# shiinamiyuki/akari_render

Hardware: AMD Instinct MI355X
Metric: Msamples/s (whole node), 1080p path tracer, C2 (higher is better)
Workload: dtype f32

## Files before the change

akari_render_amd/build.py:

```python
from __future__ import annotations

import os
import subprocess
import sys

HERE = os.path.dirname(os.path.abspath(__file__))
CSRC = os.path.join(HERE, "csrc")
LIB = os.path.join(HERE, "libakari_hip.so")

PT_KINDS = ["plain", "inst", "feat", "punct", "punct_tree"]
PT_UNITS = {"pt_unit_" + kind + ("_env" if env else "") + ("_lens" if lens else ""): 4 * k + 2 * env + lens
            for k, kind in enumerate(PT_KINDS) for env in (0, 1) for lens in (0, 1)}

SOURCES = [
    "pt_kernels.hip", "pt_kernels_relaxed.hip", *PT_UNITS, "probe_kernels.hip",
    "wf_env_kernels.hip",
    "wf_lens_kernels.hip", "aov_lens_kernels.hip",
    "wf_kernels.hip", "wf_sort.hip",
    "aov_kernels.hip", "gpt_kernels.hip", "mcmc_kernels.hip", "denoise_kernels.hip", "adapt_kernels.hip", "display_kernels.hip",
    "host/options.cpp", "host/api_common.cpp", "host/api_scene.cpp", "host/api_pt.cpp", "host/wf_schedule.cpp", "host/api_aux.cpp", "host/api_task.cpp", "host/api_probe.cpp", "host/api_denoise.cpp", "host/api_adapt.cpp", "host/api_display.cpp",
    "host/scene_build.cpp", "host/scene_inst.cpp", "host/scene_env.cpp", "host/scene_punct.cpp",
    "host/scene_json.cpp",
    "host/bvh.cpp",
    "host/image_io.cpp",
    "host/image_formats.cpp",
    "host/pmj_tables.cpp",
    "host/comm.cpp",
    "host/specialise.cpp",
]
TEST_HOOKS = os.environ.get("AKR_SHIP", "0") != "1"


def _headers():
# ... 186 lines not shown
```

akari_render_amd/capi.py:

```python
from __future__ import annotations

import ctypes as C
import os
from typing import Optional

import numpy as np

from . import abi
from .build import LIB, build

AKR_OK = 0
FILM_PLANE_RGB, FILM_PLANE_SPLAT, FILM_PLANE_WEIGHT, FILM_PLANES_PT, FILM_PLANES_ALL = 1, 2, 4, 5, 7
ERR_INVALID_ARGUMENT, ERR_HIP, ERR_NO_DEVICE, ERR_IO, ERR_PARSE, ERR_UNSUPPORTED, ERR_OOM, ERR_RENDER = -1, -2, -3, -4, -5, -6, -7, -8

(ARRAY_WOOP, ARRAY_TRI_GID, ARRAY_SHADE, ARRAY_INSTANCES, ARRAY_MATERIALS, ARRAY_BVH_NODES, ARRAY_LIGHT_ENTRIES,
 ARRAY_LIGHT_PDF, ARRAY_AREA_ENTRIES, ARRAY_AREA_PDF, ARRAY_INST_TRI_OFFSET, ARRAY_R2C, ARRAY_C2W,
 ARRAY_TEX_NODES, ARRAY_TEX_IMAGES, ARRAY_TEX_TEXELS, ARRAY_MAT_INPUTS,
 ARRAY_INST_LEAVES, ARRAY_MESH_TRIS, ARRAY_MESH_POS, ARRAY_MESH_META, ARRAY_MESH_NORMALS,
 ARRAY_ENV_MARGINAL_ENTRIES, ARRAY_ENV_MARGINAL_PDF, ARRAY_ENV_CONDITIONAL_ENTRIES, ARRAY_ENV_CONDITIONAL_PDF, ARRAY_ENV_TEXELS,
 ARRAY_PUNCTUAL_LIGHTS, ARRAY_LIGHT_TREE) = range(29)
ENV_LIGHT_INSTANCE = 0xFFFFFFFF
PUNCTUAL_LIGHT_INSTANCE = 0xFFFFFFFE
LIGHT_TREE_INSTANCE = 0xFFFFFFFD

# ... 22 lines not shown
]
TEST_EXPORTS = [
    "akr_probe_material_inputs_host", "akr_host_stdrng_u64", "akr_host_chacha_block", "akr_host_pcg32_states",
    "akr_host_pcg_start", "akr_host_alias_table", "akr_probe_math", "akr_probe_bsdf", "akr_probe_intersect",
    "akr_probe_surface_interaction", "akr_probe_material_inputs", "akr_host_decode_png", "akr_host_decode_jpeg",
    "akr_host_decode_exr", "akr_host_decode_tiff", "akr_host_decode_dds", "akr_host_pmj02bn_tables",
    "akr_probe_material_folded_host", "akr_host_sobol_dim1", "akr_host_fastmod", "akr_host_tri_pretest",
    "akr_probe_env_sample", "akr_probe_env_pdf", "akr_host_lens_ray", "akr_probe_camera_rays",
    "akr_probe_div", "akr_probe_intersect_pair", "akr_probe_math2", "akr_host_denoise", "akr_probe_denoise_times",
    "akr_host_pt_launch_plan", "akr_host_denoise_variance", "akr_probe_denoise_variance_times",
    "akr_host_tile_error", "akr_host_half_bracket", "akr_probe_adapt_times",
    "akr_host_display_transform", "akr_host_luminance_histogram", "akr_probe_display_times",
    "akr_host_pt_features_plan", "akr_host_pcg_end_pass", "akr_probe_pcg_end_pass",
    "akr_host_light_sample", "akr_probe_light_sample", "akr_host_light_sample_soft", "akr_probe_light_sample_soft",
    "akr_host_light_tree_sample", "akr_probe_light_tree_sample", "akr_host_option_info",
]


class OptionInfo(C.Structure):
    _fields_ = [("name", C.c_char_p), ("env", C.c_char_p), ("default_value", C.c_int32), ("ranged", C.c_int32), ("lo", C.c_int32), ("hi", C.c_int32)]


class RenderSession(C.Structure):

    _fields_ = [("save_intermediate", C.c_int32), ("save_stats", C.c_int32), ("name", C.c_char_p),
                ("override_sampler_independent", C.c_int32), ("verbose", C.c_int32)]


class AkariError(RuntimeError):
    def __init__(self, code: int, msg: str):
# ... 84 lines not shown
    proto("akr_film_resolve", vp, fp)
    proto("akr_film_device_ptr", vp, vpp, u64p)
    proto("akr_pt_kernel_info", vp, C.POINTER(abi.KernelInfo))
    proto("akr_scene_spec_source", vp, C.c_char_p, u64, u64p)
    proto("akr_host_spec_compile", vp, u32, u32, C.c_char_p, u64p, C.c_char_p, u32)
    proto("akr_probe_material_folded_host", vp, u32, u32, fp, up, fp, fp)
    proto("akr_host_sobol_dim1", u32, up, up, up)
    proto("akr_host_fastmod", u32, up, up, up)
    proto("akr_host_tri_pretest", u32, fp, fp, f32, up, up, fp)
    proto("akr_host_spec_compile_text", C.c_char_p, u32, u32, C.c_char_p, C.c_char_p)
    proto("akr_context_device_ordinal", vp, C.POINTER(C.c_int32))
    proto("akr_device_count", C.POINTER(C.c_int32))
    proto("akr_option_set", C.c_char_p, i32)
    proto("akr_option_get", C.c_char_p, C.POINTER(C.c_int32))
    proto("akr_host_option_info", u32, C.POINTER(OptionInfo))
    proto("akr_comm_unique_id", C.POINTER(C.c_uint8))
    proto("akr_comm_create", vp, C.POINTER(C.c_uint8), i32, i32, vpp)
    proto("akr_comm_wrap", vp, vp, i32, i32, vpp)
    proto("akr_comm_destroy", vp)
    proto("akr_film_reduce", vp, vp, i32, i32)
    proto("akr_film_reduce_planes", vp, vp, i32, i32, u32)
    proto("akr_mcmc_render_shard", vp, vp, C.POINTER(abi.McmcConfig), u32, u32, vp, C.POINTER(abi.McmcPartial), up, C.POINTER(abi.PtStats))
    proto("akr_mcmc_combine_host", vp, C.POINTER(abi.McmcPartial), u32, C.POINTER(abi.McmcResult))
    proto("akr_mcmc_combine", vp, vp, i32, C.POINTER(abi.McmcPartial), C.POINTER(abi.McmcResult))
    proto("akr_pt_config_default", C.POINTER(abi.PtConfig))
    proto("akr_aov_config_default", C.POINTER(abi.AovConfig))
    proto("akr_aov_render", vp, vp, C.POINTER(abi.AovConfig), vp, C.POINTER(abi.PtStats))
    proto("akr_gpt_config_default", C.POINTER(abi.GptConfig))
    proto("akr_gpt_render", vp, vp, C.POINTER(abi.GptConfig), vp, fp, C.POINTER(abi.PtStats))
    proto("akr_gpt_begin", vp, vp, C.POINTER(abi.GptConfig), vp, vp, vpp)
# ... 393 lines not shown


def get_option(name: str) -> int:
    v = C.c_int32()
    check(lib().akr_option_get(name.encode(), C.byref(v)))
    return v.value


def option_table() -> list:
    rows, o = [], OptionInfo()
    while lib().akr_host_option_info(len(rows), C.byref(o)) == 0:
        rows.append({"name": o.name.decode(), "env": o.env.decode(), "default": o.default_value, "range": (o.lo, o.hi) if o.ranged else None})
    return rows


class options:

    def __init__(self, **kw):
        self.kw, self.old = kw, {}

    def __enter__(self):
        for k, v in self.kw.items():
            self.old[k] = get_option(k)
            set_option(k, v)
        return self

    def __exit__(self, *exc):
        for k, v in self.old.items():
            set_option(k, v)
        return False
# ... 111 lines not shown
            self._guides = (albedo, normal)
            check(lib().akr_pt_begin_features(ctx.h if ctx is not None else None, scene.h, C.byref(self._cfg), film.h if film is not None else None,
                                              albedo.h if albedo is not None else None, normal.h if normal is not None else None, C.byref(self.h)))

    def passes(self, n: int = 1, blocking: bool = False) -> int:
        done = C.c_uint32()
        check(lib().akr_pt_passes(self.h, n, 1 if blocking else 0, C.byref(done)))
        return done.value

    def set_active_tiles(self, tiles) -> None:
        if tiles is None:
            check(lib().akr_pt_set_active_tiles(self.h, None, 0))
            return
        t = np.ascontiguousarray(tiles, dtype=np.uint32).reshape(-1)
        check(lib().akr_pt_set_active_tiles(self.h, _up(t) if t.size else C.cast(C.pointer(C.c_uint32(0)), C.POINTER(C.c_uint32)), t.size))

    def sampler_states(self, n_pixels: int) -> np.ndarray:
        st = np.zeros(2 * n_pixels, dtype=np.uint64)
        check(lib().akr_pt_read_sampler_states(self.h, st.ctypes.data_as(C.POINTER(C.c_uint64))))
        return st

    def stats(self) -> dict:
        st = abi.PtStats()
        check(lib().akr_pt_get_stats(self.h, C.byref(st)))
        return st.as_dict()

    def kernel_info(self) -> dict:
        ki = abi.KernelInfo()
        ki.struct_size = C.sizeof(abi.KernelInfo)
        check(lib().akr_pt_kernel_info(self.h, C.byref(ki)))
# ... 466 lines not shown
```

akari_render_amd/csrc/device/pt_pass.h:

```cpp
#pragma once
#include "dpath.h"

namespace akr {

#ifndef AKR_PT_MIN_WAVES
#define AKR_PT_MIN_WAVES 4
#endif
#ifndef AKR_PT_MIN_WAVES_BVH
#define AKR_PT_MIN_WAVES_BVH 4
#endif
#ifndef AKR_PT_MIN_WAVES_FD
#define AKR_PT_MIN_WAVES_FD 4
#endif
#ifndef AKR_PT_MIN_WAVES_TEX
#define AKR_PT_MIN_WAVES_TEX 3
#endif
#ifndef AKR_PT_MIN_WAVES_BVH_TEX
#define AKR_PT_MIN_WAVES_BVH_TEX 3
#endif
template <bool TEX>
using PairWalkOpt = WalkOpt<!TEX>;
template <bool BVH, bool FD, bool TEX, bool PMJ, bool STAGE, bool DEFER, uint32_t ABSENT = 0, bool INST = false, bool ENV = false, bool LENS = false, bool FEAT = false, bool PUNCT = false, bool LTREE = false>
AKR_D void pt_pass_body(const PtParams& p) {
    extern __shared__ __attribute__((aligned(16))) uint32_t lds_stack[];
// ... 11 lines not shown
        uint32_t* l = lds_stack + p.tile_offset;
        const uint32_t* g = (const uint32_t*)p.sc.bvh_nodes;
        for (uint32_t i = threadIdx.x; i < p.sc.bvh_tile_nodes * kBvhNodeWords; i += 256u) l[i] = g[i];
        __syncthreads();
    }
    const float4* lds_recs = nullptr;
    if (!BVH) {
        uint32_t* l = lds_stack + (p.stage_total >> 2);
        const uint32_t* g = (const uint32_t*)p.sc.woop;
        for (uint32_t i = threadIdx.x; i < (p.sc.n_tris + 2u) * 12u; i += 256u) l[i] = g[i];
        __syncthreads();
        lds_recs = (const float4*)l;
    }
    const uint32_t item = blockIdx.x * 256u + threadIdx.x;
    uint32_t px = 0, py = 0;
    const bool in_frame = item < p.n_items && item_to_pixel(p, item, px, py);
    const uint32_t pix = px + py * p.width;
    uint32_t sx, sy;
    shifted_pixel(p, px, py, sx, sy);
    if (PMJ && p.bn_offset != 0) pmj_bluenoise_stage(p, px, py);
    PathRegs r;
    path_regs_init<PMJ, LENS, FEAT>(r, q, in_frame, pix, sx, sy);
    constexpr bool PARK = !FD && TEX;
    uint32_t* park = lds_stack + p.park_offset + threadIdx.x;
    if (PARK) {
        park_put(park, PK_PIX, pix);
        park_put(park, PK_SX, sx);
        park_put(park, PK_SY, sy);
        if (FEAT) {
            park_put(park, PK_FEAT_A + 0, f2u(r.feat_a.x)); park_put(park, PK_FEAT_A + 1, f2u(r.feat_a.y)); park_put(park, PK_FEAT_A + 2, f2u(r.feat_a.z));
            park_put(park, PK_FEAT_N + 0, f2u(r.feat_n.x)); park_put(park, PK_FEAT_N + 1, f2u(r.feat_n.y)); park_put(park, PK_FEAT_N + 2, f2u(r.feat_n.z));
// ... 93 lines not shown
                    r.deferred = false;
                } else if (r.has_ray && found && (iteration & q.defer_metal)) {
                    const uint32_t mat = f2u(sc.shade[(size_t)hit.gid * SHADE_ROWS + 6].y);
                    if (sc.materials[mat].flags & q.defer_flags) {
                        r.d_gid = hit.gid; r.d_u = hit.u; r.d_v = hit.v;
                        r.deferred = true;
                        r.has_ray = false;
                    }
                }
            }
            if (STRAG > 0 && r.carry) {
            } else if (PARK) path_step<FD ? 1 : 0, TEX, PMJ, DEFER ? 1 : 2, ABSENT, INST, ENV, LENS, FEAT, PUNCT, LTREE>(q, r, hit, found, occluded, 0, 0, 0, park);
            else path_step<FD ? 1 : 0, TEX, PMJ, 0, ABSENT, INST, ENV, LENS, FEAT, PUNCT, LTREE>(q, r, hit, found, occluded, pix, sx, sy);
        }
    }
    flush_counters(p, r, tc.cnt, BVH);
}

constexpr int pt_pass_min_waves(bool bvh, bool fd, bool tex) {
    return bvh ? (tex ? AKR_PT_MIN_WAVES_BVH_TEX : AKR_PT_MIN_WAVES_BVH) : (fd ? AKR_PT_MIN_WAVES_FD : (tex ? AKR_PT_MIN_WAVES_TEX : AKR_PT_MIN_WAVES));
}

}
```

akari_render_amd/csrc/host/api_internal.h:

```cpp
#pragma once
#include <atomic>
#include <mutex>
#include <hip/hip_runtime.h>

#include <algorithm>
#include <array>
#include <cstdlib>
#include <cstdio>
#include <chrono>
#include <cstring>
#include <functional>
#include <map>
#include <memory>
#include <new>
#include <stdexcept>
#include <string>
#include <vector>

#include "scene_build.h"
#include "specialise.h"
#include "stdrng.h"


namespace akr_api {
// ... 164 lines not shown
struct RenderBase {
    akr_context* ctx = nullptr;
    akr_scene* scene = nullptr;
    akr_film* film = nullptr;
    akr_pt_config cfg;
    DevBuf states, counters;
    TileGrid grid;
    DevBuf owned_tiles;
    uint32_t spp_done = 0, n_launches = 0;
    uint32_t pmj_spp = 1;
    const akr_scene::ColorSet* color_set = nullptr;
    TuningOptions opt;
    std::vector<std::pair<hipEvent_t, hipEvent_t>> pending;
    double kernel_ms = 0.0;
    PtVariant variant{};
    PtParams params;
    bool holds_scene = false;
    akr_film *feat_albedo = nullptr, *feat_normal = nullptr;
    void fold_events(bool all) {
        size_t keep = 0;
        for (size_t i = 0; i < pending.size(); i++) {
            auto& ev = pending[i];
            if (all || hipEventQuery(ev.second) == hipSuccess) {
                float t = 0.0f;
                if (hipEventElapsedTime(&t, ev.first, ev.second) == hipSuccess) kernel_ms += t;
                (void)hipEventDestroy(ev.first);
                (void)hipEventDestroy(ev.second);
            } else {
                pending[keep++] = ev;
            }
// ... 27 lines not shown
    }
};

struct akr_pt_session : RenderBase {
    std::unique_ptr<WavefrontState> wf;
    int sched_trial = 0;
    uint64_t passes_launched = 0;
    bool spec_active = false;
    bool wf_sort = false;
    bool arith_relaxed = false;
    int spec_waves = 3;
    std::shared_ptr<SpecKernel> spec;
    std::string spec_status = "not requested";
    DevBuf active_tiles;
    bool active_set = false;
};

namespace akr_api {
bool choose_wavefront(const akr_pt_session* se);
std::unique_ptr<WavefrontState> wf_allocate(const akr_pt_session* se, bool sort);
void wf_set_range(WavefrontState& ws, uint32_t n_active);
void wf_run(akr_pt_session* se);
bool schedule_trial_eligible(const akr_pt_session* se);
struct LaunchTimer {
    RenderBase* se;
    hipEvent_t e0 = nullptr, e1 = nullptr;
    explicit LaunchTimer(RenderBase* s) : se(s) {
        HIP_CHECK(hipEventCreate(&e0));
        HIP_CHECK(hipEventCreate(&e1));
        HIP_CHECK(hipEventRecord(e0, se->ctx->stream));
// ... 12 lines not shown
    }
};

void base_begin(RenderBase* se, akr_context* ctx, akr_scene* scene, const akr_pt_config* cfg, akr_film* film, const TuningOptions* opt = nullptr);
int32_t render_begin(akr_context* ctx, akr_scene* scene, const akr_pt_config* cfg, akr_film* film, RenderBase** out);
int32_t base_end(RenderBase* se, akr_pt_stats* stats);
void session_params(RenderBase* se, bool spec_active = false, int spec_waves = 3);
inline void set_launch_passes(RenderBase* se, uint32_t n_passes, uint32_t last_pass_spp) {
    se->params.n_passes = n_passes;
    se->params.last_pass_spp = last_pass_spp;
}
struct PtPlan {
    PtVariant v;
    uint32_t simple_scene, defer_metal, defer_flags;
    uint32_t stage_bytes[13], stage_total, tex_slots;
};
PtPlan pt_plan(const akr_scene* s, const akr_pt_config& c, const TuningOptions& opt, bool spec_active, int spec_waves, bool feat = false);
std::string pt_features_refusal(const akr_scene* s, const TuningOptions& t);
PtVariant pt_scene_facts(const akr_scene* s, const akr_pt_config& c);
std::string pt_punctual_refusal(const akr_scene* s, const TuningOptions& t);
inline uint32_t scene_stack_depth(const CompiledScene& cs) {
    return cs.instanced.on ? cs.bvh_depth : std::max(1u, std::min(cs.bvh_depth, kBvhStackDepth));
}
inline uint32_t scene_n_nodes(const CompiledScene& cs) { return (uint32_t)((cs.instanced.on ? cs.instanced.nodes.size() : cs.bvh_nodes.size()) / kBvhNodeWords); }
void camera_params(PtParams& p, const akr_scene* s, uint32_t filter_type, float filter_radius);
template <typename End>
int32_t end_keeping_first_error(int32_t rc, End&& end) {
    const std::string err = g_last_error;
    const int32_t rc2 = end();
    if (rc == AKR_OK) return rc2;
    g_last_error = err;
    return rc;
// ... 11 lines not shown
```

akari_render_amd/csrc/host/api_probe.cpp:

```cpp
#if defined(AKR_TEST_HOOKS) && AKR_TEST_HOOKS
#include "api_internal.h"
#include "../../../include/akari_hip_test.h"
#include "../device/dinst.h"
#include "../device/disect.h"
#include "../device/dpath.h"

extern "C" {

AKR_TEST_API int32_t akr_host_stdrng_u64(uint64_t seed, uint32_t n, uint64_t* out) {
    if (!out) return fail(AKR_ERR_INVALID_ARGUMENT, "out is NULL");
    StdRng rng(seed);
    for (uint32_t i = 0; i < n; i++) out[i] = rng.next_u64();
    return AKR_OK;
}
AKR_TEST_API int32_t akr_host_chacha_block(const uint32_t* key8, uint64_t counter, uint64_t stream, int32_t rounds, uint32_t* out16) {
    if (!key8 || !out16) return fail(AKR_ERR_INVALID_ARGUMENT, "NULL argument");
    StdRng::chacha_block(key8, counter, stream, rounds, out16);
    return AKR_OK;
}
AKR_TEST_API int32_t akr_host_pcg32_states(uint64_t seed, uint64_t n, uint64_t* out2n) {
    if (!out2n) return fail(AKR_ERR_INVALID_ARGUMENT, "out is NULL");
    StdRng rng(seed);
    for (uint64_t i = 0; i < n; i++) {
        Pcg32 p = pcg_new_seq_offset(i, rng.next_u64());
// ... 345 lines not shown
        const auto vl = fill_launch_plan(scene, cfg, t, spec_waves, feat != 0, &out->plan);
        out->feat = vl.first.feat ? 1u : 0u;
        out->kernel_compiled = pt_variant_compiled(vl.first) ? 1u : 0u;
        out->park_slots = (vl.second.carry_offset - vl.second.park_offset) / 256u;
        out->required_bytes = (uint32_t)vl.second.required_bytes;
        out->lds_budget = (uint32_t)pt_lds_budget(vl.first.tex);
        out->park_slots_feat = kParkSlotsFeat;
    });
}
AKR_TEST_API int32_t akr_host_option_info(uint32_t index, akr_option_info* out) {
    OptionInfo o;
    if (!out || !tuning_info(index, &o)) return fail(AKR_ERR_INVALID_ARGUMENT, "akr_host_option_info: out is NULL or index is past the table's last row");
    *out = {o.name, o.env, o.def, o.ranged, o.lo, o.hi};
    return AKR_OK;
}
AKR_TEST_API int32_t akr_probe_camera_rays(akr_context* ctx, akr_scene* scene, uint32_t filter_type, float filter_radius, uint32_t n, const uint32_t* pixels2,
                                      const float* u4, float* out6) {
    if (!ctx || !scene || !pixels2 || !u4 || !out6) return fail(AKR_ERR_INVALID_ARGUMENT, "akr_probe_camera_rays: NULL argument");
    if (filter_type > AKR_FILTER_GAUSSIAN) return fail(AKR_ERR_INVALID_ARGUMENT, "akr_probe_camera_rays: unknown filter_type");
    return guarded([&] {
        ctx->bind();
        DevBuf dpx, du, dout;
        dpx.upload(std::vector<uint32_t>(pixels2, pixels2 + 2ull * n));
        du.upload(std::vector<float>(u4, u4 + 4ull * n));
        dout.alloc(6ull * n * 4);
        if (n) HIP_CHECK(launch_probe_camera_rays(probe_camera_params(scene, filter_type, filter_radius), n, dpx.as<uint32_t>(), du.as<float>(), dout.as<float>(), ctx->stream));
        HIP_CHECK(hipStreamSynchronize(ctx->stream));
        if (n) HIP_CHECK(hipMemcpy(out6, dout.p, 6ull * n * 4, hipMemcpyDeviceToHost));
    });
}
// ... 169 lines not shown
```

akari_render_amd/csrc/host/api_pt.cpp:

```cpp
#include "api_internal.h"

void akr_api::camera_params(PtParams& p, const akr_scene* s, uint32_t filter_type, float filter_radius) {
    std::memcpy(p.r2c, s->r2c, 64);
    std::memcpy(p.c2w, s->c2w, 64);
    p.c2w_identity = s->c2w_identity;
    p.width = s->flat.camera.width;
    p.height = s->flat.camera.height;
    p.filter_type = filter_type;
    p.filter_radius = filter_radius;
    p.lens_radius = s->flat.lens.radius;
    p.lens_focal = s->flat.lens.focal_distance;
}
PtVariant akr_api::pt_scene_facts(const akr_scene* s, const akr_pt_config& c) {
    const CompiledScene& cs = s->cs;
    PtVariant v;
    v.bvh = cs.has_tree();
    v.fd = c.force_diffuse != 0;
    v.tex = cs.has_textures;
    v.pmj = c.sampler_type != AKR_SAMPLER_INDEPENDENT;
    v.inst = cs.instanced.on;
    v.env = cs.env.on;
    v.lens = s->flat.lens.radius > 0.0f;
    v.punct = !cs.punct.empty();
    v.ltree = !cs.punct_tree.empty();
// ... 3 lines not shown
    if (s->cs.punct.empty()) return "";
    const std::string who = "a " + punctual_light_name(s->cs);
    if (t.wavefront == 1) return "unsupported: the scene has " + who + " and the wavefront schedule is forced (option wavefront = 1); only the megakernel samples punctual lights";
    if (t.arith == 1) return "unsupported: the scene has " + who + "; the relaxed arithmetic tier (option arith = 1) has no kernels that sample punctual lights";
    return "";
}
std::string akr_api::pt_features_refusal(const akr_scene* s, const TuningOptions& t) {
    if (s->cs.instanced.on)
        return "unsupported: akr_pt_begin_features: the scene is kept as meshes + instances (option instancing); its kernels collect no guides -- render them with akr_aov_render";
    if (t.wavefront == 1) return "unsupported: akr_pt_begin_features: the wavefront schedule is forced (option wavefront = 1); only the megakernel collects guides";
    if (t.arith == 1) return "unsupported: akr_pt_begin_features: the relaxed arithmetic tier (option arith = 1) has no kernels that collect guides";
    if (!s->cs.punct.empty())
        return "unsupported: akr_pt_begin_features: the scene has a " + punctual_light_name(s->cs) + "; the kernels that sample punctual lights collect no guides -- render them with akr_aov_render";
    return "";
}
PtPlan akr_api::pt_plan(const akr_scene* s, const akr_pt_config& c, const TuningOptions& opt, bool spec_active, int spec_waves, bool feat) {
    const CompiledScene& cs = s->cs;
    PtPlan pl{};
    PtVariant& v = pl.v = pt_scene_facts(s, c);
    v.feat = feat;
    const bool plain = !v.env && !v.lens && !v.feat && !v.punct;
    {
        bool simple = !cs.has_textures;
        for (const DMaterial& m : cs.materials) {
            if (m.kind == MAT_GLASS) simple = false;
            if (m.kind == MAT_PRINCIPLED && ((m.flags & (MF_COAT | MF_EVAL_DIEL | MF_NORMAL_MAP)) != 0 || m.transmission != 0.0f || m.coat_weight != 0.0f)) simple = false;
        }
        pl.simple_scene = (simple && opt.simple_kernels && plain) ? 1u : 0u;
        v.simple = pl.simple_scene != 0 && !v.fd && !v.tex && !v.inst;
    }
    {
// ... 32 lines not shown
        };
        const bool may = !v.inst && total <= (bvh ? kStageMaxBytesBvh : kStageMaxBytes);
        const size_t ggx_bytes = 4096 * sizeof(float);
        if (may && !bvh && v.tex && !v.fd && fits(total + ggx_bytes)) {
            bytes[12] = ggx_bytes;
            total += ggx_bytes;
            v.stage = true;
        } else {
            v.stage = may && (!bvh || fits(total));
        }
        if (v.stage) {
            for (int i = 0; i < 13; i++) pl.stage_bytes[i] = (uint32_t)bytes[i];
            pl.stage_total = (uint32_t)std::max<size_t>(total, 16);
        }
    }
    if (!pt_variant_compiled(v)) throw RenderError("pt_plan: no kernel for the variant decided");
    return pl;
}
void akr_api::session_params(RenderBase* se, bool spec_active, int spec_waves) {
    PtParams& p = se->params;
    const akr_scene* s = se->scene;
    const akr_pt_config& c = se->cfg;
    std::memset(&p, 0, sizeof p);
    p.sc = s->dscene;
    camera_params(p, s, c.filter_type, c.filter_radius);
    p.max_depth = c.max_depth;
    p.rr_depth = c.rr_depth;
    p.use_nee = c.use_nee;
    p.indirect_only = c.indirect_only;
    p.force_diffuse = c.force_diffuse;
// ... 19 lines not shown
    }
    p.sampler = c.sampler_type;
    if (c.sampler_type == AKR_SAMPLER_PMJ02BN || c.sampler_type == AKR_SAMPLER_SOBOL) {
        p.smp_seed = (uint32_t)c.sampler_seed;
        p.smp_spp = se->pmj_spp;
        uint32_t w = se->pmj_spp - 1;
        w |= w >> 1; w |= w >> 2; w |= w >> 4; w |= w >> 8; w |= w >> 16;
        p.smp_w = w;
        p.smp_mod_magic = fastmod_magic(se->pmj_spp);
        if (c.sampler_type == AKR_SAMPLER_PMJ02BN) {
            p.pmj_sets = se->ctx->pmj_sets.as<uint32_t>();
            p.bluenoise = se->ctx->bluenoise.as<uint16_t>();
        }
    }
    {
        const PtPlan plan = pt_plan(s, c, se->opt, spec_active, spec_waves, se->feat_albedo != nullptr);
        se->variant = plan.v;
        std::memcpy(p.stage_bytes, plan.stage_bytes, sizeof p.stage_bytes);
        p.stage_total = plan.stage_total;
        p.tex_slots = plan.tex_slots;
        p.simple_scene = plan.simple_scene;
        p.defer_metal = plan.defer_metal;
        p.defer_flags = plan.defer_flags;
    }
    for (int a = 0; a < 3; a++) {
        const float lo = s->cs.scene_lo[a], ext = s->cs.scene_hi[a] - s->cs.scene_lo[a];
        p.sort_lo[a] = lo;
        p.sort_scale[a] = ext > 0.0f ? 128.0f / ext : 0.0f;
    }
    p.shard_rank = c.shard_count > 1 ? c.shard_rank : 0;
    p.shard_count = c.shard_count > 1 ? c.shard_count : 1;
    p.tile_w = se->grid.tile_w;
// ... 6 lines not shown
    p.feat_normal = se->feat_normal ? se->feat_normal->data : nullptr;
}
std::vector<uint32_t> akr_api::owned_tiles(uint32_t tiles_x, uint32_t tiles_y, uint32_t rank, uint32_t count) {
    std::vector<std::pair<uint32_t, uint32_t>> mine;
    for (uint32_t ty = 0; ty < tiles_y; ty++)
        for (uint32_t tx = 0; tx < tiles_x; tx++)
            if (tile_owner(tx, ty, count) == rank) mine.emplace_back(tile_morton(tx, ty), ty * tiles_x + tx);
    std::sort(mine.begin(), mine.end());
    std::vector<uint32_t> out;
    out.reserve(mine.size());
    for (const auto& m : mine) out.push_back(m.second);
    return out;
}

static void read_stats(RenderBase* se, akr_pt_stats* stats);

static void validate_config(const akr_pt_config& c, const TileGrid& grid) {
    if (c.spp_per_pass == 0) throw std::invalid_argument("akr_pt_config: spp_per_pass must be > 0");
    if (c.filter_type > AKR_FILTER_GAUSSIAN) throw std::invalid_argument("akr_pt_config: unknown filter_type");
    if (c.sampler_type > AKR_SAMPLER_SOBOL) throw std::invalid_argument("akr_pt_config: unknown sampler_type");
    if (c.color > (AKR_COLOR_REPR_ACESCG | AKR_COLOR_RGB_ACESCG)) throw std::invalid_argument("akr_pt_config: unknown colour pipeline bits");
    if (c.sampler_type == AKR_SAMPLER_PMJ02BN && c.spp > 65536u)
        throw std::invalid_argument("Pmj02BnSampler supports up to 65536 spp (sampler/mod.rs:381-387)");
    if ((grid.tile_w % 8) || (grid.tile_h % 8)) throw std::invalid_argument("akr_pt_config: tile_w and tile_h must be multiples of 8");
    if (c.shard_count > 1 && c.shard_rank >= c.shard_count) throw std::invalid_argument("akr_pt_config: shard_rank >= shard_count");
    if (c.sample_begin != 0 || c.sample_count != 0) {
        if (c.sampler_type != AKR_SAMPLER_PMJ02BN && c.sampler_type != AKR_SAMPLER_SOBOL)
            throw Unsupported("akr_pt_config: a sample range needs an index-based sampler (pmj02bn, sobol): the independent sampler's start() advances the pixel's "
                              "PCG stream from wherever the previous sample stopped (sampler/mod.rs:115-131,192-203), sample s cannot be drawn without samples 0 .. s-1");
        if (c.sample_count == 0) throw std::invalid_argument("akr_pt_config: sample_begin without sample_count");
// ... 68 lines not shown
        se->states.upload(init);
    } else {
        std::vector<uint64_t> seeds(n);
        StdRng rng(cfg->sampler_seed);
        for (auto& v : seeds) v = rng.next_u64();
        DevBuf dseeds;
        dseeds.upload(seeds);
        se->states.alloc(n * sizeof(Pcg32));
        HIP_CHECK(launch_init_pcg32(dseeds.as<uint64_t>(), se->states.p, n, ctx->stream));
        HIP_CHECK(hipStreamSynchronize(ctx->stream));
    }
    se->counters.alloc(8 * kStatStripes * sizeof(uint64_t));
    HIP_CHECK(hipMemsetAsync(se->counters.p, 0, se->counters.bytes, ctx->stream));
    if (cfg->shard_count > 1) se->owned_tiles.upload(owned_tiles(se->grid.tiles_x, se->grid.tiles_y, cfg->shard_rank, cfg->shard_count));
    se->opt = opt ? *opt : tuning();
    scene->sessions++;
    se->holds_scene = true;
}
int32_t akr_api::render_begin(akr_context* ctx, akr_scene* scene, const akr_pt_config* cfg, akr_film* film, RenderBase** out) {
    *out = nullptr;
    return guarded([&] {
        auto se = std::make_unique<RenderBase>();
        base_begin(se.get(), ctx, scene, cfg, film);
        session_params(se.get());
        HIP_CHECK(hipStreamSynchronize(ctx->stream));
        *out = se.release();
    });
}
static int32_t pt_begin(akr_context* ctx, akr_scene* scene, const akr_pt_config* cfg, akr_film* film, akr_film* albedo, akr_film* normal, const TuningOptions& t, akr_pt_session** out) {
    *out = nullptr;
// ... 37 lines not shown
                se->spec_waves = t.specialise_waves ? t.specialise_waves : 3;
                se->spec_active = true;
            }
            session_params(se.get(), se->spec_active, se->spec_waves);
            if (se->spec_active) {
                se->spec = ctx->spec_cache.get(scene->spec_header, se->variant, se->spec_waves, ctx->props.gcnArchName, may_compile);
                se->spec_status = se->spec->status;
                if (!se->spec->fn) {
                    se->spec_active = false;
                    session_params(se.get(), false, se->spec_waves);
                }
            }
            se->params.wf_sort = se->wf_sort ? 1u : 0u;
        }
        if (wavefront) se->wf = wf_allocate(se.get(), se->wf_sort);
        se->sched_trial = schedule_trial_eligible(se.get()) ? 1 : 0;
        HIP_CHECK(hipStreamSynchronize(ctx->stream));
        *out = se.release();
    });
}
extern "C" {
AKR_API int32_t akr_pt_begin(akr_context* ctx, akr_scene* scene, const akr_pt_config* cfg, akr_film* film, akr_pt_session** out) {
    if (!out) return fail(AKR_ERR_INVALID_ARGUMENT, "akr_pt_begin: NULL argument");
    return pt_begin(ctx, scene, cfg, film, nullptr, nullptr, tuning(), out);
}
AKR_API int32_t akr_pt_begin_features(akr_context* ctx, akr_scene* scene, const akr_pt_config* cfg, akr_film* film, akr_film* albedo, akr_film* normal, akr_pt_session** out) {
    if (!out) return fail(AKR_ERR_INVALID_ARGUMENT, "akr_pt_begin_features: NULL argument");
    *out = nullptr;
    if (!ctx || (scene && !scene->ctx))
        return fail(AKR_ERR_UNSUPPORTED, "unsupported: akr_pt_begin_features: guides are collected by GPU kernels; a host-only scene (no device context) cannot render them");
// ... 4 lines not shown
        if (g->ctx != ctx) return fail(AKR_ERR_INVALID_ARGUMENT, "akr_pt_begin_features: a guide film belongs to another context");
        if (g->width != scene->flat.camera.width || g->height != scene->flat.camera.height)
            return fail(AKR_ERR_INVALID_ARGUMENT, "akr_pt_begin_features: a guide film's resolution does not match the scene camera");
    }
    const TuningOptions t = tuning();
    const std::string why = pt_features_refusal(scene, t);
    if (!why.empty()) return fail(AKR_ERR_UNSUPPORTED, why);
    return pt_begin(ctx, scene, cfg, film, albedo, normal, t, out);
}
AKR_API int32_t akr_pt_passes(akr_pt_session* se, uint32_t n_passes, int32_t blocking, uint32_t* spp_done) {
    if (!se) return fail(AKR_ERR_INVALID_ARGUMENT, "session is NULL");
    return guarded([&] {
        se->ctx->bind();
        uint32_t kMaxFusedPasses = 16;
        se->fold_events(false);
        if (se->opt.max_fused_passes > 0) {
            kMaxFusedPasses = (uint32_t)se->opt.max_fused_passes;
        } else if (blocking && se->pending.empty() && se->passes_launched > 0 && se->kernel_ms > 0.0) {
            const double per_pass_ms = se->kernel_ms / (double)se->passes_launched;
            const double fit = 3000.0 / per_pass_ms;
            kMaxFusedPasses = fit >= 64.0 ? 64u : (fit <= 16.0 ? 16u : (uint32_t)fit);
        }
        uint32_t left = n_passes;
        const uint32_t total = session_samples(se->cfg);
        auto launch = [&](uint32_t max_fused) {
            uint32_t fused = 0, last = 0, done = se->spp_done;
            while (fused < max_fused && fused < left && done < total) {
                last = std::min(total - done, se->cfg.spp_per_pass);
                done += last;
                fused++;
            }
            set_launch_passes(se, fused, last);
            LaunchTimer timer(se);
            if (se->active_set && se->params.n_items == 0) {}
            else if (se->wf) wf_run(se);
            else HIP_CHECK(launch_pt_pass(se->params, se->variant, se->ctx->stream, se->spec_active ? se->spec->fn : nullptr, se->arith_relaxed));
            timer.stop();
            se->spp_done = done;
            se->n_launches++;
            se->passes_launched += fused;
            left -= fused;
        };
        if (se->sched_trial == 1 && blocking && left >= 4 && total - se->spp_done >= 4 * se->cfg.spp_per_pass) {
            se->sched_trial = 2;
            auto timed = [&](double& ms_per_sample, double& shaded_per_closest) {
                HIP_CHECK(hipStreamSynchronize(se->ctx->stream));
                akr_pt_stats a, b;
                read_stats(se, &a);
                launch(2);
                read_stats(se, &b);
                ms_per_sample = (b.kernel_ms - a.kernel_ms) / (double)std::max<uint64_t>(1, b.n_samples - a.n_samples);
// ... 29 lines not shown
        const uint32_t n_tiles = se->grid.tiles_x * se->grid.tiles_y, tile_px = se->grid.tile_w * se->grid.tile_h;
        const uint32_t count = c.shard_count > 1 ? c.shard_count : 1, rank = c.shard_count > 1 ? c.shard_rank : 0;
        if (tiles) {
            std::vector<uint8_t> seen(n_tiles, 0);
            for (uint32_t j = 0; j < n; j++) {
                const uint32_t t = tiles[j];
                if (t >= n_tiles) throw std::invalid_argument("akr_pt_set_active_tiles: tile " + std::to_string(t) + " is out of range (the grid has " + std::to_string(n_tiles) + " tiles)");
                if (tile_owner(t % se->grid.tiles_x, t / se->grid.tiles_x, count) != rank)
                    throw std::invalid_argument("akr_pt_set_active_tiles: tile " + std::to_string(t) + " is not owned by this session (shard " + std::to_string(rank) + " of " + std::to_string(count) + ")");
                if (seen[t]) throw std::invalid_argument("akr_pt_set_active_tiles: duplicate tile " + std::to_string(t));
                seen[t] = 1;
            }
        }
        HIP_CHECK(hipStreamSynchronize(se->ctx->stream));
        se->sched_trial = se->sched_trial == 1 ? 0 : se->sched_trial;
        if (!tiles) {
            se->active_set = false;
            p.shard_count = count;
            p.owned_tiles = se->owned_tiles.as<uint32_t>();
            p.n_items = se->grid.n_items;
        } else {
            if (!se->active_tiles.p) se->active_tiles.alloc((size_t)std::max(1u, n_tiles) * sizeof(uint32_t));
            if (n) HIP_CHECK(hipMemcpy(se->active_tiles.p, tiles, (size_t)n * sizeof(uint32_t), hipMemcpyHostToDevice));
            se->active_set = true;
            p.shard_count = std::max(2u, count);
            p.owned_tiles = se->active_tiles.as<uint32_t>();
            p.n_items = n * tile_px;
        }
        if (se->wf) wf_set_range(*se->wf, p.n_items);
    });
// ... 46 lines not shown
        info->struct_size = size;
        info->specialised = se->spec_active ? 1u : 0u;
        info->n_shader_kinds = (uint32_t)se->scene->cs.shader_kinds.size();
        const PtVariant& v = se->variant;
        info->kernel_flags = (v.bvh && !v.inst ? 1u : 0u) | (v.pmj ? 2u : 0u) | (v.stage ? 4u : 0u) | (v.defer ? 8u : 0u) | (se->arith_relaxed ? 16u : 0u) | (v.lens ? 32u : 0u) | (v.feat ? 64u : 0u) | (v.punct ? 128u : 0u) |
                             (v.ltree ? 256u : 0u);
        info->absent_mask = se->scene->cs.absent;
        if (se->spec) {
            info->cache_hit = se->spec->cache_hit ? 1u : 0u;
            info->min_waves = (uint32_t)se->spec_waves;
            info->vgprs = (uint32_t)se->spec->vgprs;
            info->scratch_bytes = (uint32_t)se->spec->scratch_bytes;
            info->compile_ms = se->spec->compile_ms;
            info->load_ms = se->spec->load_ms;
        }
        std::snprintf(info->status, sizeof info->status, "%s", se->spec_status.c_str());
        if (se->wf && se->wf->buf.carry != nullptr && se->counters.p) {
            const uint64_t carried = read_counters(se)[7];
            std::snprintf(info->status, sizeof info->status, "%s; %llu rays carried into a later trace launch", se->spec_status.c_str(), (unsigned long long)carried);
        }
    });
}
AKR_API int32_t akr_pt_end(akr_pt_session* se, akr_pt_stats* stats) { return base_end(se, stats); }
AKR_API int32_t akr_pt_render(akr_context* ctx, akr_scene* scene, const akr_pt_config* cfg, akr_film* film, akr_pt_stats* stats) {
    akr_pt_session* se = nullptr;
    int32_t rc = akr_pt_begin(ctx, scene, cfg, film, &se);
    if (rc != AKR_OK) return rc;
    uint32_t n_passes = (session_samples(*cfg) + cfg->spp_per_pass - 1) / cfg->spp_per_pass;
    rc = akr_pt_passes(se, n_passes, 1, nullptr);
    return end_keeping_first_error(rc, [&] { return akr_pt_end(se, stats); });
}
// ... 18 lines not shown
```

akari_render_amd/csrc/kernels.h:

```cpp
#pragma once
#if !defined(__HIPCC_RTC__)
#include <hip/hip_runtime.h>
#endif

#include "device/drng.h"
#include "device/dscene.h"

#if !defined(__HIPCC_RTC__)
#include <algorithm>
struct PtVariant {
    bool bvh = false, fd = false, tex = false, pmj = false, stage = false, defer = false, simple = false, inst = false, env = false, lens = false;
    bool feat = false;
    bool punct = false;
    bool ltree = false;
};
constexpr bool pt_variant_compiled(const PtVariant& v) {
    return (v.bvh || v.stage) && !(v.defer && (v.fd || (v.bvh && !v.tex))) && !(v.simple && (v.fd || v.tex)) && !((v.env || v.lens || v.feat || v.punct) && (v.defer || v.simple)) &&
           !(v.inst && !(v.bvh && !v.stage && !v.defer && !v.simple && !v.feat)) && !(v.punct && (v.feat || v.inst)) && !(v.ltree && !v.punct);
}
constexpr uint32_t pt_variant_bits(const PtVariant& v) {
    return (v.bvh ? 1u : 0u) | (v.pmj ? 2u : 0u) | (v.stage ? 4u : 0u) | (v.defer ? 8u : 0u) | (v.inst ? 16u : 0u) | (v.env ? 32u : 0u) | (v.lens ? 64u : 0u) |
           (v.feat ? 128u : 0u) | (v.punct ? 256u : 0u) | (v.ltree ? 512u : 0u);
}
constexpr PtVariant pt_variant_from_bits(uint32_t f) {
// ... 143 lines not shown
    uint32_t stage_total;
    uint32_t simple_scene;
    uint32_t defer_metal;
    uint32_t defer_flags;
    uint32_t tex_slots;
    uint32_t tile_offset;
    uint32_t park_offset;
    uint32_t carry_offset;
    uint32_t bn_offset;
    uint32_t wf_sort;
    float sort_lo[3], sort_scale[3];
    uint32_t n_items;
    uint32_t shard_rank, shard_count;
    uint32_t tile_w, tile_h, tiles_x, tiles_y;
    const uint32_t* owned_tiles;
    float lens_radius, lens_focal;
    float *feat_albedo, *feat_normal;
};

AKR_HD uint32_t morton_spread16(uint32_t x) {
    x &= 0xffffu;
    x = (x | (x << 8)) & 0x00ff00ffu;
    x = (x | (x << 4)) & 0x0f0f0f0fu;
    x = (x | (x << 2)) & 0x33333333u;
    x = (x | (x << 1)) & 0x55555555u;
    return x;
}
AKR_HD uint32_t tile_morton(uint32_t tx, uint32_t ty) { return morton_spread16(tx) | (morton_spread16(ty) << 1); }
AKR_HD uint32_t tile_owner(uint32_t tx, uint32_t ty, uint32_t count) { return tile_morton(tx, ty) % count; }

// ... 81 lines not shown
hipError_t launch_probe_light_sample(const PtParams& p, uint32_t n, const float* rows9, float* out13, uint32_t* light, hipStream_t stream);
hipError_t launch_probe_light_tree_sample(const PtParams& p, uint32_t n, const float* rows9, float* out13, uint32_t* light, uint32_t* record, hipStream_t stream);
hipError_t launch_probe_camera_rays(const PtParams& p, uint32_t n, const uint32_t* pixels2, const float* u4, float* out6, hipStream_t stream);
hipError_t launch_pt_pass(const PtParams& p, const PtVariant& v, hipStream_t stream, hipFunction_t spec_fn = nullptr, bool relaxed = false);
hipError_t launch_gpt_sample(const PtParams& p, const GptParams& g, hipStream_t stream);
hipError_t launch_gpt_update(const GptParams& g, uint32_t W, uint32_t H, float* film, hipStream_t stream);
hipError_t launch_gpt_recon_init(const GptParams& g, uint32_t W, uint32_t H, float* old, float spp, hipStream_t stream);
hipError_t launch_gpt_recon(const GptParams& g, uint32_t W, uint32_t H, const float* old, float* cur, float scaling, float spp, hipStream_t stream);
hipError_t launch_aov(const PtParams& p, uint32_t spp, uint32_t aov, uint32_t remap, hipStream_t stream);
hipError_t launch_wf_init(const PtParams& p, const WfBuffers& wf, hipStream_t stream);
hipError_t launch_wf_shade(const PtParams& p, const WfBuffers& wf, uint32_t q_out, hipStream_t stream);
uint32_t wf_trace_blocks_per_cu(const PtParams& p);
hipError_t launch_wf_trace(const PtParams& p, const WfBuffers& wf, uint32_t q_in, uint32_t n_blocks, hipStream_t stream);
size_t wf_sort_temp_bytes(uint32_t n);
hipError_t wf_sort_pairs(void* temp, size_t temp_bytes, const uint32_t* keys_in, uint32_t* keys_out, const uint32_t* vals_in, uint32_t* vals_out, uint32_t n, hipStream_t stream);
hipError_t launch_probe_material(const PtParams& p, uint32_t material, uint32_t n, const float* uv, uint32_t* out, hipStream_t stream);
hipError_t launch_init_pcg32(const uint64_t* seeds, void* states, uint64_t n, hipStream_t stream);
hipError_t launch_film_resolve(const float* film, uint64_t n, float splat_scale, float* rgb, hipStream_t stream);
hipError_t launch_ggx_table(const uint64_t* seeds, float* table, uint32_t samples, hipStream_t stream);
hipError_t launch_probe_math(uint32_t n, const float* x, float* s, float* c, float* l, hipStream_t stream);
hipError_t launch_probe_math2(uint32_t n, const float* xy, float* out, hipStream_t stream);
hipError_t launch_probe_bsdf(const DMaterial* m, const float* table, int mode, const float* wo, uint32_t n, const float* in, float* out,
                             hipStream_t stream);
hipError_t launch_probe_div(uint32_t n, const float* a, const float* b, float* out_fast, float* out_ieee, hipStream_t stream);
hipError_t launch_probe_pcg_end_pass(uint32_t n, const uint64_t* state, const uint64_t* inc, const uint32_t* dim, uint64_t* out_closed, uint64_t* out_loop, hipStream_t stream);
hipError_t launch_probe_intersect_pair(const PtParams& p, uint32_t n, const float* rays, const uint32_t* excl, uint32_t* out, float* out_tuv, hipStream_t stream);
hipError_t launch_probe_intersect(const PtParams& p, uint32_t n, const float* rays, uint32_t* out, float* bary, hipStream_t stream);
hipError_t launch_probe_si(const PtParams& p, uint32_t n, const uint32_t* inst_prim, const float* bary, float* out, hipStream_t stream);
#endif

// ... 2 lines not shown
```

Measured before the change: 3490.

## Reorder megakernel work items by recorded per-pixel cost after first pass

Result: faster. 3676 (median of 6 runs) (+5.3%).

```diff
diff --git a/akari_render_amd/build.py b/akari_render_amd/build.py
--- a/akari_render_amd/build.py
+++ b/akari_render_amd/build.py
@@ -17,6 +17,7 @@
     "wf_env_kernels.hip",
     "wf_lens_kernels.hip", "aov_lens_kernels.hip",
     "wf_kernels.hip", "wf_sort.hip",
+    "cost_order_kernels.hip",
     "aov_kernels.hip", "gpt_kernels.hip", "mcmc_kernels.hip", "denoise_kernels.hip", "adapt_kernels.hip", "display_kernels.hip",
     "host/options.cpp", "host/api_common.cpp", "host/api_scene.cpp", "host/api_pt.cpp", "host/wf_schedule.cpp", "host/api_aux.cpp", "host/api_task.cpp", "host/api_probe.cpp", "host/api_denoise.cpp", "host/api_adapt.cpp", "host/api_display.cpp",
     "host/scene_build.cpp", "host/scene_inst.cpp", "host/scene_env.cpp", "host/scene_punct.cpp",
diff --git a/akari_render_amd/capi.py b/akari_render_amd/capi.py
--- a/akari_render_amd/capi.py
+++ b/akari_render_amd/capi.py
@@ -60,6 +60,7 @@
     "akr_host_pt_features_plan", "akr_host_pcg_end_pass", "akr_probe_pcg_end_pass",
     "akr_host_light_sample", "akr_probe_light_sample", "akr_host_light_sample_soft", "akr_probe_light_sample_soft",
     "akr_host_light_tree_sample", "akr_probe_light_tree_sample", "akr_host_option_info",
+    "akr_probe_pt_cost_order", "akr_probe_pt_cost_order_mode",
 ]
 
 
@@ -174,6 +175,8 @@
     proto("akr_option_set", C.c_char_p, i32)
     proto("akr_option_get", C.c_char_p, C.POINTER(C.c_int32))
     proto("akr_host_option_info", u32, C.POINTER(OptionInfo))
+    proto("akr_probe_pt_cost_order", vp, up, up, up, u32, up, fp)
+    proto("akr_probe_pt_cost_order_mode", i32, C.POINTER(C.c_int32))
     proto("akr_comm_unique_id", C.POINTER(C.c_uint8))
     proto("akr_comm_create", vp, C.POINTER(C.c_uint8), i32, i32, vpp)
     proto("akr_comm_wrap", vp, vp, i32, i32, vpp)
@@ -597,6 +600,20 @@
     return rows
 
 
+class cost_order_mode:
+
+    def __init__(self, mode: int):
+        self.mode, self.old = int(mode), C.c_int32(1)
+
+    def __enter__(self):
+        check(lib().akr_probe_pt_cost_order_mode(self.mode, C.byref(self.old)))
+        return self
+
+    def __exit__(self, *exc):
+        check(lib().akr_probe_pt_cost_order_mode(self.old.value, None))
+        return False
+
+
 class options:
 
     def __init__(self, **kw):
@@ -738,6 +755,15 @@
             return
         t = np.ascontiguousarray(tiles, dtype=np.uint32).reshape(-1)
         check(lib().akr_pt_set_active_tiles(self.h, _up(t) if t.size else C.cast(C.pointer(C.c_uint32(0)), C.POINTER(C.c_uint32)), t.size))
+
+    def cost_order(self, n_pixels: int) -> dict:
+        state, n_table, ms = C.c_uint32(), C.c_uint32(), C.c_float()
+        check(lib().akr_probe_pt_cost_order(self.h, C.byref(state), None, None, 0, C.byref(n_table), None))
+        cost = np.zeros(n_pixels, dtype=np.uint32) if state.value or n_table.value else None
+        table = np.zeros(n_table.value, dtype=np.uint32)
+        check(lib().akr_probe_pt_cost_order(self.h, C.byref(state), _up(cost) if cost is not None else None, _up(table) if table.size else None, table.size,
+                                            C.byref(n_table), C.byref(ms)))
+        return {"state": state.value, "cost": cost, "table": table, "sort_ms": ms.value}
 
     def sampler_states(self, n_pixels: int) -> np.ndarray:
         st = np.zeros(2 * n_pixels, dtype=np.uint64)
diff --git a/akari_render_amd/csrc/cost_order_kernels.hip b/akari_render_amd/csrc/cost_order_kernels.hip
--- /dev/null
+++ b/akari_render_amd/csrc/cost_order_kernels.hip
@@ -0,0 +1,55 @@
+#include <hip/hip_runtime.h>
+#include <cstring>
+#include <rocprim/device/device_radix_sort.hpp>
+
+#include "device/dpath.h"
+
+namespace akr {
+
+__global__ __launch_bounds__(256) void k_cost_order_keys(const PtParams p, uint32_t n_padded, uint64_t* __restrict__ keys) {
+    const uint32_t item = blockIdx.x * 256u + threadIdx.x;
+    if (item >= n_padded) return;
+    uint32_t px = 0, py = 0;
+    uint64_t key = ~0ull;
+    if (item < p.n_items && item_to_pixel(p, item, px, py)) {
+        const uint32_t pix = px + py * p.width;
+        key = ((uint64_t)(~p.item_cost[item]) << 32) | pix;
+    }
+    keys[item] = key;
+}
+__global__ __launch_bounds__(256) void k_cost_order_table(const uint64_t* __restrict__ keys, uint32_t n_padded, uint32_t* __restrict__ table) {
+    const uint32_t item = blockIdx.x * 256u + threadIdx.x;
+    if (item < n_padded) table[item] = (uint32_t)keys[item];
+}
+
+__global__ __launch_bounds__(256) void k_cost_to_pixels(const PtParams p, const uint32_t* __restrict__ item_cost, uint32_t* __restrict__ pixel_cost) {
+    const uint32_t item = blockIdx.x * 256u + threadIdx.x;
+    uint32_t px = 0, py = 0;
+    if (item < p.n_items && item_to_pixel(p, item, px, py)) pixel_cost[px + py * p.width] = item_cost[item];
+}
+hipError_t launch_cost_to_pixels(const PtParams& p, const uint32_t* item_cost, uint32_t* pixel_cost, hipStream_t stream) {
+    const uint32_t blocks = (p.n_items + 255u) / 256u;
+    if (blocks == 0) return hipSuccess;
+    hipLaunchKernelGGL(k_cost_to_pixels, dim3(blocks), dim3(256), 0, stream, p, item_cost, pixel_cost);
+    return hipGetLastError();
+}
+
+size_t cost_order_temp_bytes(uint32_t n_padded) {
+    size_t bytes = 0;
+    (void)rocprim::radix_sort_keys(nullptr, bytes, (const uint64_t*)nullptr, (uint64_t*)nullptr, (size_t)n_padded, 0u, 64u, (hipStream_t) nullptr);
+    return bytes;
+}
+hipError_t launch_cost_order(const PtParams& p, uint32_t n_padded, uint64_t* keys, uint64_t* keys_sorted, void* temp, size_t temp_bytes, uint32_t* table, hipStream_t stream) {
+    if (n_padded == 0) return hipSuccess;
+    if (p.item_cost == nullptr || (n_padded & 255u) != 0 || n_padded < p.n_items) return hipErrorInvalidValue;
+    const uint32_t blocks = n_padded / 256u;
+    hipLaunchKernelGGL(k_cost_order_keys, dim3(blocks), dim3(256), 0, stream, p, n_padded, keys);
+    hipError_t e = hipGetLastError();
+    if (e != hipSuccess) return e;
+    e = rocprim::radix_sort_keys(temp, temp_bytes, (const uint64_t*)keys, keys_sorted, (size_t)n_padded, 0u, 64u, stream);
+    if (e != hipSuccess) return e;
+    hipLaunchKernelGGL(k_cost_order_table, dim3(blocks), dim3(256), 0, stream, (const uint64_t*)keys_sorted, n_padded, table);
+    return hipGetLastError();
+}
+
+}
diff --git a/akari_render_amd/csrc/device/pt_pass.h b/akari_render_amd/csrc/device/pt_pass.h
--- a/akari_render_amd/csrc/device/pt_pass.h
+++ b/akari_render_amd/csrc/device/pt_pass.h
@@ -49,7 +49,14 @@
     }
     const uint32_t item = blockIdx.x * 256u + threadIdx.x;
     uint32_t px = 0, py = 0;
-    const bool in_frame = item < p.n_items && item_to_pixel(p, item, px, py);
+    bool in_frame;
+    if (p.item_pixels != nullptr) {
+        const uint32_t t = p.item_pixels[item];
+        in_frame = t != kInvalid;
+        if (in_frame) { py = t / p.width; px = t - py * p.width; }
+    } else {
+        in_frame = item < p.n_items && item_to_pixel(p, item, px, py);
+    }
     const uint32_t pix = px + py * p.width;
     uint32_t sx, sy;
     shifted_pixel(p, px, py, sx, sy);
@@ -173,6 +180,7 @@
             else path_step<FD ? 1 : 0, TEX, PMJ, 0, ABSENT, INST, ENV, LENS, FEAT, PUNCT, LTREE>(q, r, hit, found, occluded, pix, sx, sy);
         }
     }
+    if (p.item_cost != nullptr) p.item_cost[item] = r.c_closest;
     flush_counters(p, r, tc.cnt, BVH);
 }
 
diff --git a/akari_render_amd/csrc/host/api_internal.h b/akari_render_amd/csrc/host/api_internal.h
--- a/akari_render_amd/csrc/host/api_internal.h
+++ b/akari_render_amd/csrc/host/api_internal.h
@@ -202,6 +202,8 @@
     std::vector<std::pair<hipEvent_t, hipEvent_t>> pending;
     double kernel_ms = 0.0;
     PtVariant variant{};
+    int cost_order_mode = 1;
+    bool plan_cost_order = false;
     PtParams params;
     bool holds_scene = false;
     akr_film *feat_albedo = nullptr, *feat_normal = nullptr;
@@ -259,6 +261,15 @@
     std::string spec_status = "not requested";
     DevBuf active_tiles;
     bool active_set = false;
+    int cost_order = 0;
+    bool cost_recorded = false;
+    DevBuf item_cost, item_pixels, cost_keys, cost_keys_sorted, cost_sort_tmp;
+    float cost_sort_ms = 0.0f;
+    hipEvent_t cost_ev0 = nullptr, cost_ev1 = nullptr;
+    ~akr_pt_session() override {
+        if (cost_ev0) (void)hipEventDestroy(cost_ev0);
+        if (cost_ev1) (void)hipEventDestroy(cost_ev1);
+    }
 };
 
 namespace akr_api {
@@ -301,8 +312,11 @@
     PtVariant v;
     uint32_t simple_scene, defer_metal, defer_flags;
     uint32_t stage_bytes[13], stage_total, tex_slots;
-};
-PtPlan pt_plan(const akr_scene* s, const akr_pt_config& c, const TuningOptions& opt, bool spec_active, int spec_waves, bool feat = false);
+    bool cost_order;
+};
+PtPlan pt_plan(const akr_scene* s, const akr_pt_config& c, const TuningOptions& opt, bool spec_active, int spec_waves, bool feat = false, int cost_order = 1);
+int cost_order_mode();
+int cost_order_mode_set(int mode);
 std::string pt_features_refusal(const akr_scene* s, const TuningOptions& t);
 PtVariant pt_scene_facts(const akr_scene* s, const akr_pt_config& c);
 std::string pt_punctual_refusal(const akr_scene* s, const TuningOptions& t);
diff --git a/akari_render_amd/csrc/host/api_probe.cpp b/akari_render_amd/csrc/host/api_probe.cpp
--- a/akari_render_amd/csrc/host/api_probe.cpp
+++ b/akari_render_amd/csrc/host/api_probe.cpp
@@ -383,6 +383,38 @@
     *out = {o.name, o.env, o.def, o.ranged, o.lo, o.hi};
     return AKR_OK;
 }
+AKR_TEST_API int32_t akr_probe_pt_cost_order_mode(int32_t mode, int32_t* previous) {
+    if (mode < 0 || mode > 2) return fail(AKR_ERR_INVALID_ARGUMENT, "akr_probe_pt_cost_order_mode: mode must be 0, 1 or 2");
+    const int before = cost_order_mode_set(mode);
+    if (previous) *previous = before;
+    return AKR_OK;
+}
+AKR_TEST_API int32_t akr_probe_pt_cost_order(akr_pt_session* se, uint32_t* state, uint32_t* cost, uint32_t* table, uint32_t capacity, uint32_t* n_table, float* sort_ms) {
+    if (!se || !state || !n_table) return fail(AKR_ERR_INVALID_ARGUMENT, "akr_probe_pt_cost_order: NULL argument");
+    return guarded([&] {
+        se->ctx->bind();
+        HIP_CHECK(hipStreamSynchronize(se->ctx->stream));
+        *state = (uint32_t)se->cost_order;
+        *n_table = (uint32_t)(se->item_pixels.bytes / sizeof(uint32_t));
+        if (cost) {
+            if (!se->item_cost.p || se->active_set) throw std::invalid_argument("akr_probe_pt_cost_order: the session has no cost map, or renders an active-tile list");
+            DevBuf map;
+            map.alloc(se->film->n_floats() / 7 * sizeof(uint32_t));
+            HIP_CHECK(hipMemsetAsync(map.p, 0, map.bytes, se->ctx->stream));
+            HIP_CHECK(launch_cost_to_pixels(se->params, se->item_cost.as<uint32_t>(), map.as<uint32_t>(), se->ctx->stream));
+            HIP_CHECK(hipStreamSynchronize(se->ctx->stream));
+            HIP_CHECK(hipMemcpy(cost, map.p, map.bytes, hipMemcpyDeviceToHost));
+        }
+        if (table && *n_table) {
+            if (capacity < *n_table) throw std::invalid_argument("akr_probe_pt_cost_order: the table has " + std::to_string(*n_table) + " entries");
+            HIP_CHECK(hipMemcpy(table, se->item_pixels.p, se->item_pixels.bytes, hipMemcpyDeviceToHost));
+        }
+        if (sort_ms) {
+            *sort_ms = 0.0f;
+            if (se->cost_ev1) HIP_CHECK(hipEventElapsedTime(sort_ms, se->cost_ev0, se->cost_ev1));
+        }
+    });
+}
 AKR_TEST_API int32_t akr_probe_camera_rays(akr_context* ctx, akr_scene* scene, uint32_t filter_type, float filter_radius, uint32_t n, const uint32_t* pixels2,
                                       const float* u4, float* out6) {
     if (!ctx || !scene || !pixels2 || !u4 || !out6) return fail(AKR_ERR_INVALID_ARGUMENT, "akr_probe_camera_rays: NULL argument");
diff --git a/akari_render_amd/csrc/host/api_pt.cpp b/akari_render_amd/csrc/host/api_pt.cpp
--- a/akari_render_amd/csrc/host/api_pt.cpp
+++ b/akari_render_amd/csrc/host/api_pt.cpp
@@ -41,7 +41,10 @@
         return "unsupported: akr_pt_begin_features: the scene has a " + punctual_light_name(s->cs) + "; the kernels that sample punctual lights collect no guides -- render them with akr_aov_render";
     return "";
 }
-PtPlan akr_api::pt_plan(const akr_scene* s, const akr_pt_config& c, const TuningOptions& opt, bool spec_active, int spec_waves, bool feat) {
+static std::atomic<int> g_cost_order_mode{1};
+int akr_api::cost_order_mode() { return g_cost_order_mode.load(); }
+int akr_api::cost_order_mode_set(int mode) { return mode >= 0 && mode <= 2 ? g_cost_order_mode.exchange(mode) : g_cost_order_mode.load(); }
+PtPlan akr_api::pt_plan(const akr_scene* s, const akr_pt_config& c, const TuningOptions& opt, bool spec_active, int spec_waves, bool feat, int cost_order) {
     const CompiledScene& cs = s->cs;
     PtPlan pl{};
     PtVariant& v = pl.v = pt_scene_facts(s, c);
@@ -104,6 +107,7 @@
             pl.stage_total = (uint32_t)std::max<size_t>(total, 16);
         }
     }
+    pl.cost_order = cost_order == 2 || (cost_order == 1 && !v.bvh && !v.tex && !v.inst && !v.feat);
     if (!pt_variant_compiled(v)) throw RenderError("pt_plan: no kernel for the variant decided");
     return pl;
 }
@@ -153,8 +157,9 @@
         }
     }
     {
-        const PtPlan plan = pt_plan(s, c, se->opt, spec_active, spec_waves, se->feat_albedo != nullptr);
+        const PtPlan plan = pt_plan(s, c, se->opt, spec_active, spec_waves, se->feat_albedo != nullptr, se->cost_order_mode);
         se->variant = plan.v;
+        se->plan_cost_order = plan.cost_order;
         std::memcpy(p.stage_bytes, plan.stage_bytes, sizeof p.stage_bytes);
         p.stage_total = plan.stage_total;
         p.tex_slots = plan.tex_slots;
@@ -191,6 +196,29 @@
 }
 
 static void read_stats(RenderBase* se, akr_pt_stats* stats);
+
+static void cost_order_drop(akr_pt_session* se) {
+    se->cost_order = 0;
+    se->params.item_cost = nullptr;
+    se->params.item_pixels = nullptr;
+}
+static void cost_order_build(akr_pt_session* se) {
+    PtParams& p = se->params;
+    const uint32_t n_padded = (p.n_items + 255u) & ~255u;
+    se->item_pixels.alloc((size_t)n_padded * sizeof(uint32_t));
+    se->cost_keys.alloc((size_t)n_padded * sizeof(uint64_t));
+    se->cost_keys_sorted.alloc((size_t)n_padded * sizeof(uint64_t));
+    se->cost_sort_tmp.alloc(std::max<size_t>(16, cost_order_temp_bytes(n_padded)));
+    HIP_CHECK(hipEventCreate(&se->cost_ev0));
+    HIP_CHECK(hipEventCreate(&se->cost_ev1));
+    HIP_CHECK(hipEventRecord(se->cost_ev0, se->ctx->stream));
+    HIP_CHECK(launch_cost_order(p, n_padded, se->cost_keys.as<uint64_t>(), se->cost_keys_sorted.as<uint64_t>(), se->cost_sort_tmp.p, se->cost_sort_tmp.bytes,
+                                se->item_pixels.as<uint32_t>(), se->ctx->stream));
+    HIP_CHECK(hipEventRecord(se->cost_ev1, se->ctx->stream));
+    p.item_pixels = se->item_pixels.as<uint32_t>();
+    p.item_cost = nullptr;
+    se->cost_order = 2;
+}
 
 static void validate_config(const akr_pt_config& c, const TileGrid& grid) {
     if (c.spp_per_pass == 0) throw std::invalid_argument("akr_pt_config: spp_per_pass must be > 0");
@@ -289,6 +317,7 @@
     HIP_CHECK(hipMemsetAsync(se->counters.p, 0, se->counters.bytes, ctx->stream));
     if (cfg->shard_count > 1) se->owned_tiles.upload(owned_tiles(se->grid.tiles_x, se->grid.tiles_y, cfg->shard_rank, cfg->shard_count));
     se->opt = opt ? *opt : tuning();
+    se->cost_order_mode = cost_order_mode();
     scene->sessions++;
     se->holds_scene = true;
 }
@@ -356,6 +385,12 @@
             se->params.wf_sort = se->wf_sort ? 1u : 0u;
         }
         if (wavefront) se->wf = wf_allocate(se.get(), se->wf_sort);
+        if (se->plan_cost_order && !wavefront && !se->arith_relaxed) {
+            se->item_cost.alloc((size_t)((se->grid.n_items + 255u) & ~255u) * sizeof(uint32_t));
+            if (se->item_cost.p) HIP_CHECK(hipMemsetAsync(se->item_cost.p, 0, se->item_cost.bytes, ctx->stream));
+            se->params.item_cost = se->item_cost.as<uint32_t>();
+            se->cost_order = 1;
+        }
         se->sched_trial = schedule_trial_eligible(se.get()) ? 1 : 0;
         HIP_CHECK(hipStreamSynchronize(ctx->stream));
         *out = se.release();
@@ -390,6 +425,11 @@
         se->ctx->bind();
         uint32_t kMaxFusedPasses = 16;
         se->fold_events(false);
+        if (se->cost_order == 2 && se->cost_keys.p && se->pending.empty()) {
+            se->cost_keys.release();
+            se->cost_keys_sorted.release();
+            se->cost_sort_tmp.release();
+        }
         if (se->opt.max_fused_passes > 0) {
             kMaxFusedPasses = (uint32_t)se->opt.max_fused_passes;
         } else if (blocking && se->pending.empty() && se->passes_launched > 0 && se->kernel_ms > 0.0) {
@@ -409,8 +449,14 @@
             set_launch_passes(se, fused, last);
             LaunchTimer timer(se);
             if (se->active_set && se->params.n_items == 0) {}
-            else if (se->wf) wf_run(se);
-            else HIP_CHECK(launch_pt_pass(se->params, se->variant, se->ctx->stream, se->spec_active ? se->spec->fn : nullptr, se->arith_relaxed));
+            else if (se->wf) {
+                if (se->cost_order) cost_order_drop(se);
+                wf_run(se);
+            } else {
+                if (se->cost_order == 1 && se->cost_recorded && se->params.n_items > 0) cost_order_build(se);
+                se->cost_recorded = se->cost_recorded || se->cost_order == 1;
+                HIP_CHECK(launch_pt_pass(se->params, se->variant, se->ctx->stream, se->spec_active ? se->spec->fn : nullptr, se->arith_relaxed));
+            }
             timer.stop();
             se->spp_done = done;
             se->n_launches++;
@@ -470,6 +516,7 @@
         }
         HIP_CHECK(hipStreamSynchronize(se->ctx->stream));
         se->sched_trial = se->sched_trial == 1 ? 0 : se->sched_trial;
+        if (se->cost_order) cost_order_drop(se);
         if (!tiles) {
             se->active_set = false;
             p.shard_count = count;
@@ -546,7 +593,8 @@
             info->compile_ms = se->spec->compile_ms;
             info->load_ms = se->spec->load_ms;
         }
-        std::snprintf(info->status, sizeof info->status, "%s", se->spec_status.c_str());
+        const char* order = se->cost_order == 2 ? "; cost order: in use" : (se->cost_order == 1 ? "; cost order: recording" : "");
+        std::snprintf(info->status, sizeof info->status, "%s%s", se->spec_status.c_str(), order);
         if (se->wf && se->wf->buf.carry != nullptr && se->counters.p) {
             const uint64_t carried = read_counters(se)[7];
             std::snprintf(info->status, sizeof info->status, "%s; %llu rays carried into a later trace launch", se->spec_status.c_str(), (unsigned long long)carried);
diff --git a/akari_render_amd/csrc/kernels.h b/akari_render_amd/csrc/kernels.h
--- a/akari_render_amd/csrc/kernels.h
+++ b/akari_render_amd/csrc/kernels.h
@@ -181,6 +181,8 @@
     uint32_t shard_rank, shard_count;
     uint32_t tile_w, tile_h, tiles_x, tiles_y;
     const uint32_t* owned_tiles;
+    uint32_t* item_cost;
+    const uint32_t* item_pixels;
     float lens_radius, lens_focal;
     float *feat_albedo, *feat_normal;
 };
@@ -292,6 +294,9 @@
 hipError_t launch_wf_trace(const PtParams& p, const WfBuffers& wf, uint32_t q_in, uint32_t n_blocks, hipStream_t stream);
 size_t wf_sort_temp_bytes(uint32_t n);
 hipError_t wf_sort_pairs(void* temp, size_t temp_bytes, const uint32_t* keys_in, uint32_t* keys_out, const uint32_t* vals_in, uint32_t* vals_out, uint32_t n, hipStream_t stream);
+size_t cost_order_temp_bytes(uint32_t n_padded);
+hipError_t launch_cost_order(const PtParams& p, uint32_t n_padded, uint64_t* keys, uint64_t* keys_sorted, void* temp, size_t temp_bytes, uint32_t* table, hipStream_t stream);
+hipError_t launch_cost_to_pixels(const PtParams& p, const uint32_t* item_cost, uint32_t* pixel_cost, hipStream_t stream);
 hipError_t launch_probe_material(const PtParams& p, uint32_t material, uint32_t n, const float* uv, uint32_t* out, hipStream_t stream);
 hipError_t launch_init_pcg32(const uint64_t* seeds, void* states, uint64_t n, hipStream_t stream);
 hipError_t launch_film_resolve(const float* film, uint64_t n, float splat_scale, float* rgb, hipStream_t stream);
```
